# Blaizzy/mlx-audio

Measured on AMD Instinct MI355X. Metric: audio samples/sec + real-time factor, Kokoro-82M TTS, higher is better.
Workload: dtype bf16 weights x fp32 activations: vocoder convs = fp16 hi pass (v_mfma_f32_32x32x16_f16) + block-scaled FP4 (e2m1) lo pass (v_mfma_scale_f32_32x32x64_f8f6f4 cbsz / blgp 4, OCP MX: E8M0 scale per row x 32 channels / per output column), fp32 accumulate; front end bf16 hi+lo split; 1 GPU; Kokoro-82M bf16 TTS, tokens->waveform, canonical short sentence T=80 F=264 (6.6 s @ 24 kHz); utterances_per_gpu=64, global_batch=64, samples_per_utterance=158400, parallelism=utterance-dp1, precision_mode=6, wire=fp32

## Files before the change

include/mi355audio.h:

```cpp
#ifndef MI355AUDIO_H
#define MI355AUDIO_H

#include <stdint.h>

#ifdef __cplusplus
extern "C" {
#endif

#define MI355_OK 0
#define MI355_ERR_ARG (-1)
#define MI355_ERR_LAUNCH (-2)
#define MI355_ERR_UNSUPPORTED (-3)

const char* mi355_last_error(void);
int mi355_abi_version(void);
int mi355_device_info(int dev, char* name, int name_cap, int* cu_count, int* lds_bytes);

enum { MI355_ACT_NONE = 0, MI355_ACT_LEAKY = 1, MI355_ACT_SNAKE = 2, MI355_ACT_GELU = 3,
       MI355_ACT_ELU = 4,
       MI355_ACT_SILU = 5,
       MI355_ACT_GELU_TANH = 6,
       MI355_ACT_TANH = 7 };

typedef struct {
// ... 66 lines not shown
int mi355_pack_conv_weight_mx4_host(const float* w_host, int32_t Cout, int32_t K, int32_t Cin, uint8_t* out_host);

typedef struct {
  const float* x; int64_t x_bstride; int32_t ldx; int32_t C; int32_t L; const int32_t* lens;
  int32_t B;
  double* sums;
  const float* gb;
  int32_t gb_ld;
  float eps;
  float* scale; float* shift; int32_t out_ld;
  int32_t reuse_sums;
} mi355_adain_coef_args;
int mi355_adain_coef(const mi355_adain_coef_args* a, void* stream);

typedef struct {
  const float* partials; int64_t bstride;
  int32_t C; int32_t L; const int32_t* lens; int32_t B;
  const float* gb; int32_t gb_ld; float eps;
  float* scale; float* shift; int32_t out_ld;
} mi355_adain_partials_args;
int mi355_adain_from_partials(const mi355_adain_partials_args* a, void* stream);

typedef struct {
  const float* x; int64_t x_bstride; int32_t ldx;
  const float* res; int64_t res_bstride; int32_t ldr;
  int32_t C; int32_t L; const int32_t* lens; int32_t B;
  const float* weight; const float* bias;
  const float* ada_gb; int32_t ada_ld;
  float eps;
  int32_t post_act; float post_slope;
  float* y; int64_t y_bstride; int32_t ldy;
  int32_t y_split;
} mi355_layernorm_args;
int mi355_layernorm(const mi355_layernorm_args* a, void* stream);
int mi355_split16(const float* x, void* y, int64_t n, int32_t fmt, void* stream);

#define MI355_GN_PART_ELEMS 4096
typedef struct {
  const float* x; int64_t x_bstride; int32_t ldx;
  int32_t C; int32_t L; const int32_t* lens; int32_t B;
  double* partials; int64_t partials_bstride;
} mi355_group_norm_stats_args;
int mi355_group_norm_stats(const mi355_group_norm_stats_args* a, void* stream);

typedef struct {
  const void* partials; int64_t partials_bstride;
// ... 250 lines not shown
  const float* x; int64_t x_bstride; int32_t ldx; int32_t Fr; const int32_t* lens; int32_t B;
  int32_t n_fft; int32_t hop; const float* window;
  float* audio; int32_t ld_audio;
} mi355_istft_head_args;
int mi355_istft_head(const mi355_istft_head_args* a, void* stream);

typedef struct {
  const float* x; int64_t x_bstride; int32_t ldx; int32_t Cin; int32_t L; const int32_t* lens; int32_t B;
  const uint16_t* w; const float* bias; int32_t Cout; int32_t K; int32_t dil; int32_t pad;
  int32_t pre_act; float pre_slope; int32_t precision;
  int32_t n_fft; int32_t hop; const float* window;
  float* audio; int32_t ld_audio;
} mi355_conv_post_istft_args;
int mi355_conv_post_istft(const mi355_conv_post_istft_args* a, void* stream);

typedef struct {
  const float* x; int64_t x_bstride; int32_t ldx; int32_t Cin; int32_t L; const int32_t* lens; int32_t B;
  const uint16_t* w; const float* bias; int32_t Cout; int32_t K; int32_t u; int32_t p; int32_t row_off;
  float slope; int32_t precision;
  const float* res; int64_t res_bstride; int32_t ldr;
  float* y; int64_t y_bstride; int32_t ldy;
} mi355_upsample_polyphase_args;
int mi355_upsample_polyphase(const mi355_upsample_polyphase_args* a, void* stream);

typedef struct {
  const float* x; int32_t ldx; int32_t L; int32_t B;
  int32_t n_fft; int32_t hop; const float* window;
  int32_t pad_mode; int32_t n_frames;
  float* out;
} mi355_stft_args;
int mi355_stft(const mi355_stft_args* a, void* stream);

typedef struct {
  const float* x; int32_t ldx; int32_t L; int32_t B;
  int32_t n_fft; int32_t hop; const float* window; int32_t pad_mode; int32_t n_frames;
  const float* fb; int32_t n_mels; int32_t mode;
  float* out;
  float* gmax;
  float log_guard;
} mi355_logmel_args;
int mi355_logmel(const mi355_logmel_args* a, void* stream);
int mi355_logmel_finish(float* y, int64_t n_per_item, const float* gmax, int32_t B, void* stream);

typedef struct {
  const float* x; int32_t L;
  int32_t win; int32_t shift; int32_t pad; int32_t n_fft; int32_t n_frames;
// ... 426 lines not shown
```

mlx_audio_amd/csrc/norm.hip:

```cpp
#include "common.h"

namespace {

__global__ __launch_bounds__(256) void instnorm_partial_kernel(const mi355_adain_coef_args a, int rows_per_split) {
  __shared__ double red[2][32][33];
  const int tid = threadIdx.x, cg = tid & 7, rg = tid >> 3;
  const int b = blockIdx.z, c = blockIdx.x * 32 + cg * 4;
  const int len = a.lens ? a.lens[b] : a.L;
  const int r0 = blockIdx.y * rows_per_split;
  const int r1 = min(len, r0 + rows_per_split);
  double s[4] = {0, 0, 0, 0}, q[4] = {0, 0, 0, 0};
  const float* xb = a.x + (int64_t)b * a.x_bstride;
  if (c < a.C) {
    for (int l = r0 + rg; l < r1; l += 32) {
      const float4 v = *(const float4*)(xb + (int64_t)l * a.ldx + c);
      const float t[4] = {v.x, v.y, v.z, v.w};
#pragma unroll
      for (int i = 0; i < 4; ++i) { const double d = (double)t[i]; s[i] += d; q[i] += d * d; }
    }
  }
#pragma unroll
  for (int i = 0; i < 4; ++i) { red[0][rg][cg * 4 + i] = s[i]; red[1][rg][cg * 4 + i] = q[i]; }
  __syncthreads();
  if (tid < 64) {
// ... 89 lines not shown
        const float2 v0 = *(const float2*)(pb + (int64_t)e * estride), v1 = *(const float2*)(pb + (int64_t)(e + LPC) * estride);
        m2 += term(v0, e) + term(v1, e + LPC);
      }
      for (; e < nblk; e += LPC) m2 += term(*(const float2*)(pb + (int64_t)e * estride), e);
    }
  }
  red[cl][eg] = m2;
  __syncthreads();
  if (eg != 0 || c >= a.out_ld) return;
  float sc = 0.f, sh = 0.f;
  if (cok) {
    double q = 0.0;
    for (int j = 0; j < LPC; ++j) q += red[cl][j];
    double var = len > 0 ? q / (double)len : 0.0;
    if (var < 0) var = 0;
    const float rstd = 1.0f / sqrtf((float)var + a.eps);
    float g = 0.f, be = 0.f;
    if (a.gb) { g = a.gb[(int64_t)b * a.gb_ld + c]; be = a.gb[(int64_t)b * a.gb_ld + a.C + c]; }
    sc = (1.0f + g) * rstd;
    sh = be - (float)mean * sc;
  }
  a.scale[(int64_t)b * a.out_ld + c] = sc;
  a.shift[(int64_t)b * a.out_ld + c] = sh;
}

template <bool VEC, int NCH>
__global__ __launch_bounds__(256) void layernorm_kernel(const mi355_layernorm_args a) {
  const int lane = threadIdx.x & 63;
  const int64_t row = (int64_t)blockIdx.x * 4 + (threadIdx.x >> 6);
  if (row >= (int64_t)a.B * a.L) return;
  const int b = (int)(row / a.L), l = (int)(row - (int64_t)b * a.L);
  const int len = a.lens ? a.lens[b] : a.L;
  if (l >= len) return;
  const float* xr = a.x + (int64_t)b * a.x_bstride + (int64_t)l * a.ldx;
  const float* rr = a.res ? a.res + (int64_t)b * a.res_bstride + (int64_t)l * a.ldr : nullptr;
  float v[NCH][4];
  float s = 0.f;
  float4 w4[NCH], b4[NCH], g4[NCH], e4[NCH];
#pragma unroll
  for (int i = 0; i < NCH; ++i) {
    const int c = i * 256 + lane * 4;
    w4[i] = make_float4(1.f, 1.f, 1.f, 1.f); b4[i] = make_float4(0.f, 0.f, 0.f, 0.f); g4[i] = b4[i]; e4[i] = b4[i];
    if (c < a.C) {
      auto ld4 = [](const float* p) {
        if constexpr (VEC) return *(const float4*)p;
        else return make_float4(p[0], p[1], p[2], p[3]);
// ... 90 lines not shown
    MI355_CLEAR_ERROR();
    hipLaunchKernelGGL(instnorm_partial_kernel, dim3(cblocks, nsplit, a.B), dim3(256), 0, st, a, rows);
    MI355_LAUNCH_CHECK("instnorm_partial");
  }
  MI355_CLEAR_ERROR();
  hipLaunchKernelGGL(adain_finalize_kernel, dim3((a.out_ld + 127) / 128, a.B), dim3(128), 0, st, a);
  MI355_LAUNCH_CHECK("adain_finalize");
  return MI355_OK;
}

extern "C" int mi355_adain_from_partials(const mi355_adain_partials_args* ap, void* stream) {
  MI355_REQUIRE(ap && ap->partials && ap->scale && ap->shift, "adain_from_partials: null tensor");
  const mi355_adain_partials_args a = *ap;
  MI355_REQUIRE(a.B > 0 && a.C > 0 && a.L > 0 && a.out_ld >= a.C, "adain_from_partials: bad shape");
  MI355_CLEAR_ERROR();
  MI355_REQUIRE(a.bstride % 2 == 0 && ((uintptr_t)a.partials) % 8 == 0, "adain_from_partials: partials must be 8-byte aligned");
  static const int cpw_env = getenv("MI355_ADAIN_CPW") ? atoi(getenv("MI355_ADAIN_CPW")) : 0;
  if (a.B >= 8 && cpw_env != 4) hipLaunchKernelGGL(adain_from_partials_kernel<16>, dim3((a.out_ld + 15) / 16, a.B), dim3(256), 0, (hipStream_t)stream, a);
  else hipLaunchKernelGGL(adain_from_partials_kernel<4>, dim3((a.out_ld + 3) / 4, a.B), dim3(256), 0, (hipStream_t)stream, a);
  MI355_LAUNCH_CHECK("adain_from_partials");
  return MI355_OK;
}

extern "C" int mi355_layernorm(const mi355_layernorm_args* ap, void* stream) {
  MI355_REQUIRE(ap && ap->x && ap->y, "layernorm: null tensor");
  const mi355_layernorm_args a = *ap;
  MI355_REQUIRE(a.C > 0 && a.C <= 2048 && a.C % 4 == 0, "layernorm: C must be a multiple of 4 and <= 2048 (got %d)", a.C);
  MI355_REQUIRE(a.ldx % 4 == 0 && a.ldy % 4 == 0 && a.x_bstride % 4 == 0 && a.y_bstride % 4 == 0, "layernorm: strides must be multiples of 4");
  MI355_REQUIRE(!a.res || (a.ldr % 4 == 0 && a.res_bstride % 4 == 0), "layernorm: residual strides must be multiples of 4");
  MI355_REQUIRE(a.y_split == 0 || a.y_split == 2 || a.y_split == 4, "layernorm: y_split must be 0, 2 or 4");
  const int64_t rows = (int64_t)a.B * a.L;
  MI355_CLEAR_ERROR();
  const bool vec = ((uintptr_t)a.weight % 16 == 0) && ((uintptr_t)a.bias % 16 == 0) && ((uintptr_t)a.ada_gb % 16 == 0) && (a.ada_ld % 4 == 0);
  const dim3 grid((unsigned)((rows + 3) / 4));
  if (a.C <= 1024) {
    if (vec) hipLaunchKernelGGL((layernorm_kernel<true, 4>), grid, dim3(256), 0, (hipStream_t)stream, a);
    else hipLaunchKernelGGL((layernorm_kernel<false, 4>), grid, dim3(256), 0, (hipStream_t)stream, a);
  } else {
    if (vec) hipLaunchKernelGGL((layernorm_kernel<true, 8>), grid, dim3(256), 0, (hipStream_t)stream, a);
    else hipLaunchKernelGGL((layernorm_kernel<false, 8>), grid, dim3(256), 0, (hipStream_t)stream, a);
  }
  MI355_LAUNCH_CHECK("layernorm");
  return MI355_OK;
}
```

mlx_audio_amd/csrc/upsample_poly.hip:

```cpp
#include "conv_common.h"

using namespace mi355conv;

namespace {

constexpr int kUpThreads = 512;

template <int CIN, int COUT, int U, int MF, int NF>
__global__ __launch_bounds__(kUpThreads, 4) void upsample_poly_kernel(const mi355_upsample_polyphase_args a, const int nblk) {
  constexpr int H = MF * 32, R = H + 1, NCH = CIN / 32;
  constexpr int CHB = R * 64;
  constexpr int PLANE = NCH * CHB;
  constexpr int NFRAG = U * COUT / 32;
  constexpr int NG = NFRAG / NF;
  constexpr int NTp = ((U * COUT + 127) >> 7) << 2;
  constexpr int64_t WSTEP = (int64_t)NTp * 2048;
  constexpr int NS = NCH * 2;
  constexpr int DEPTH = 3;
  static_assert(NFRAG % NF == 0 && (COUT / 32) % NF == 0, "a column group lies inside one phase");
  static_assert(H * NCH * 8 % kUpThreads == 0, "whole passes over the first H window rows");
  extern __shared__ __attribute__((aligned(16))) char smem[];
  char* const A_hi = smem;
  char* const A_lo = smem + PLANE;

  const int tid = threadIdx.x;
  const int b = (int)blockIdx.x / nblk;
  const int m0 = ((int)blockIdx.x - b * nblk) * H;
  const int len_raw = a.lens ? a.lens[b] : a.L;
  const int len_in = len_raw < 0 ? 0 : (len_raw > a.L ? a.L : len_raw);
  if (m0 > len_in) return;
  const int len_up = len_in * U;

// ... 24 lines not shown
#pragma unroll
        for (int j = 0; j < 4; ++j) {
          float u = in[j] + 0.0f;
          const float m = u * slope;
          u = u > 0.f ? u : m;
          tt[j] = rowok ? u : 0.f;
        }
        uint2 ph, pl;
        ph.x = pack_bf16x2(tt[0], tt[1]);
        ph.y = pack_bf16x2(tt[2], tt[3]);
        const float h0 = __builtin_bit_cast(float, ph.x << 16), h1 = __builtin_bit_cast(float, ph.x & 0xffff0000u);
        const float h2 = __builtin_bit_cast(float, ph.y << 16), h3 = __builtin_bit_cast(float, ph.y & 0xffff0000u);
        pl.x = pack_bf16x2(tt[0] - h0, tt[1] - h1);
        pl.y = pack_bf16x2(tt[2] - h2, tt[3] - h3);
        const int addr = chunk * CHB + r * 64 + ((((c4 >> 3) ^ ((r >> 2) & 3))) << 4) + ((c4 & 4) << 1);
        *(uint2*)(A_hi + addr) = ph;
        *(uint2*)(A_lo + addr) = pl;
      }
    }
  }
  float* const yb = a.y + (int64_t)b * a.y_bstride;
  const float* const rb = a.res + (int64_t)b * a.res_bstride;
  if (a.row_off && m0 == 0) {
    for (int c = tid; c < COUT; c += kUpThreads) yb[c] = rb[c];
  }
  __syncthreads();

  const int wave = __builtin_amdgcn_readfirstlane(tid >> 6);
  for (int g = wave; g < NG; g += kUpThreads / 64) {
    int lane = tid & 63;
    asm volatile("" : "+v"(lane));
    const int hl = lane & 31, hh = lane >> 5;
    const int f0 = g * NF;
    const int phase = (f0 * 32) / COUT, oc0 = f0 * 32 - phase * COUT;
    const int nc0 = m0 * U + phase - a.p;
    const int len_up_c = len_up > 0 ? len_up : 1;

    f32x16 acc[MF][NF];
#pragma unroll
    for (int mf = 0; mf < MF; ++mf)
#pragma unroll
      for (int nf = 0; nf < NF; ++nf)
#pragma unroll
        for (int r = 0; r < 16; ++r) acc[mf][nf][r] = 0.f;

    const char* const wfrag = (const char*)a.w + (int64_t)f0 * 2048 + lane * 16;
    bf16x8 ring[DEPTH][2 * NF];
// ... 15 lines not shown
        bf16x8 ah[MF], al[MF];
#pragma unroll
        for (int mf = 0; mf < MF; ++mf) {
          const int row = mf * 32 + hl + tap;
          const int addr = chunk * CHB + row * 64 + (((kk * 2 + hh) ^ ((row >> 2) & 3)) << 4);
          ah[mf] = *(const bf16x8*)(A_hi + addr);
          al[mf] = *(const bf16x8*)(A_lo + addr);
        }
#pragma unroll
        for (int mf = 0; mf < MF; ++mf) {
#pragma unroll
          for (int nf = 0; nf < NF; ++nf) acc[mf][nf] = mfma16<2>(ah[mf], ring[sl % DEPTH][2 * nf + kk], acc[mf][nf]);
#pragma unroll
          for (int nf = 0; nf < NF; ++nf) acc[mf][nf] = mfma16<2>(al[mf], ring[sl % DEPTH][2 * nf + kk], acc[mf][nf]);
        }
      }
    }

    {
      const uint32_t col = (uint32_t)(oc0 + hl) * 4u, ypb = (uint32_t)a.ldy * 4u, rpb = (uint32_t)a.ldr * 4u;
      float bias[NF];
#pragma unroll
      for (int nf = 0; nf < NF; ++nf) bias[nf] = a.bias ? a.bias[oc0 + nf * 32 + hl] : 0.f;
#pragma unroll
      for (int mf = 0; mf < MF; ++mf) {
        float rv[NF][16];
#pragma unroll
        for (int r = 0; r < 16; ++r) {
          int nc = nc0 + (mf * 32 + (r & 3) + 8 * (r >> 2) + 4 * hh) * U;
          nc = nc < 0 ? 0 : (nc >= len_up_c ? len_up_c - 1 : nc);
          const uint32_t off = (uint32_t)(nc + a.row_off) * rpb + col;
#pragma unroll
          for (int nf = 0; nf < NF; ++nf) rv[nf][r] = *(const float*)((const char*)rb + (off + (uint32_t)(nf * 128)));
        }
#pragma unroll
        for (int r = 0; r < 16; ++r) {
          const int nc = nc0 + (mf * 32 + (r & 3) + 8 * (r >> 2) + 4 * hh) * U;
          if (nc >= 0 && nc < len_up) {
            const uint32_t off = (uint32_t)(nc + a.row_off) * ypb + col;
#pragma unroll
            for (int nf = 0; nf < NF; ++nf) *(float*)((char*)yb + (off + (uint32_t)(nf * 128))) = (acc[mf][nf][r] + bias[nf]) + rv[nf][r];
          }
        }
      }
    }
  }
}

template <int CIN, int COUT, int U, int MF, int NF>
int launch_up(const mi355_upsample_polyphase_args& a, hipStream_t st) {
  constexpr int H = MF * 32;
  constexpr int lds = 2 * (CIN / 32) * (H + 1) * 64;
  static bool attr_set = false;
  if (!attr_set) {
    hipError_t e = hipFuncSetAttribute((const void*)upsample_poly_kernel<CIN, COUT, U, MF, NF>, hipFuncAttributeMaxDynamicSharedMemorySize, lds);
    MI355_REQUIRE(e == hipSuccess, "upsample_polyphase: cannot reserve %d bytes of LDS: %s", lds, hipGetErrorString(e));
    attr_set = true;
  }
  const int nblk = (a.L + 1 + H - 1) / H;
  MI355_REQUIRE((int64_t)a.B * nblk < (int64_t)1 << 31, "upsample_polyphase: too many row blocks");
  MI355_CLEAR_ERROR();
  hipLaunchKernelGGL((upsample_poly_kernel<CIN, COUT, U, MF, NF>), dim3((unsigned)(a.B * nblk)), dim3(kUpThreads), lds, st, a, nblk);
  MI355_LAUNCH_CHECK("upsample_polyphase");
  return MI355_OK;
}

}

extern "C" int mi355_upsample_polyphase(const mi355_upsample_polyphase_args* ap, void* stream) {
  MI355_REQUIRE(ap && ap->x && ap->w && ap->res && ap->y, "upsample_polyphase: null tensor");
  const mi355_upsample_polyphase_args a = *ap;
  const bool s0 = a.Cin == 512 && a.Cout == 256 && a.u == 10, s1 = a.Cin == 256 && a.Cout == 128 && a.u == 6;
  if (!(s0 || s1) || a.K != 2 * a.u || a.p != (a.K - a.u) / 2 || a.precision != 2 || (a.row_off != 0 && a.row_off != 1)) {
    mi355_set_error("upsample_polyphase: unsupported shape (Cin=%d Cout=%d u=%d K=%d p=%d row_off=%d precision=%d)", a.Cin, a.Cout, a.u, a.K, a.p,
                    a.row_off, a.precision);
    return MI355_ERR_UNSUPPORTED;
  }
  const int64_t Lo = (int64_t)a.L * a.u + a.row_off;
  MI355_REQUIRE(a.B > 0 && a.L > 0 && a.ldx >= a.Cin && a.ldr >= a.Cout && a.ldy >= a.Cout, "upsample_polyphase: bad shape");
  MI355_REQUIRE(a.B == 1 || (a.x_bstride >= (int64_t)a.L * a.ldx && a.res_bstride >= Lo * a.ldr && a.y_bstride >= Lo * a.ldy), "upsample_polyphase: items overlap");
  MI355_REQUIRE(Lo * a.ldr < ((int64_t)1 << 29) && Lo * a.ldy < ((int64_t)1 << 29), "upsample_polyphase: an item's rows exceed the 32-bit byte offsets");
  MI355_REQUIRE((a.ldx & 3) == 0 && (a.x_bstride & 3) == 0 && (((uintptr_t)a.x | (uintptr_t)a.w) & 15) == 0, "upsample_polyphase: input rows must be 16-byte aligned");
  if (s0) return launch_up<512, 256, 10, 1, 2>(a, (hipStream_t)stream);
  return launch_up<256, 128, 6, 2, 1>(a, (hipStream_t)stream);
}
```

mlx_audio_amd/ops.py:

```python
from __future__ import annotations

import ctypes
import math
import os
from dataclasses import dataclass
from typing import Optional, Tuple

import numpy as np
import torch

from . import _lib

ACT_NONE, ACT_LEAKY, ACT_SNAKE, ACT_GELU, ACT_ELU, ACT_SILU, ACT_GELU_TANH, ACT_TANH = 0, 1, 2, 3, 4, 5, 6, 7

PROFILE = None


def _stream() -> int:
    return torch.cuda.current_stream().cuda_stream


def profile_finalize(entries):
    torch.cuda.synchronize()
    out = []
    for rows, cin, cout, k, dil, extra_reads, e0, e1 in entries:
        rows = int(rows)
        flops = 2.0 * rows * cout * k * cin
        byts = 4.0 * rows * (cin + cout * (1 + extra_reads)) + 2.0 * cout * k * cin
        out.append((flops, byts, e0, e1, (cin, cout, k, dil, rows)))
# ... 1550 lines not shown
            e0, e1 = torch.cuda.Event(enable_timing=True), torch.cuda.Event(enable_timing=True)
            e0.record()
            PROFILE.append(((L * B) if lens is None else lens.sum(), pc.cin, pc.cout, pc.k, dil, 0, e0, e1))
        _lib.call_struct("mi355_conv_post_istft", "mi355_conv_post_istft_args", _stream(), x=_ptr(x), x_bstride=xbs, ldx=ldx, Cin=pc.cin, L=L,
                         lens=_ptr(lens), B=B, w=_ptr(pc.w), bias=_ptr(pc.bias), Cout=pc.cout, K=pc.k, dil=dil, pad=pad, pre_act=pre_act,
                         pre_slope=pre_slope, precision=precision, n_fft=n_fft, hop=hop, window=_ptr(window), audio=_ptr(audio),
                         ld_audio=audio.stride(0))
        if PROFILE is not None:
            e1.record()
        return audio
    post = torch.empty((B, L, round_up(pc.cout, 4)), dtype=torch.float32, device=x.device)[:, :, :pc.cout]
    conv_gemm(x, pc, post, dil=dil, pad=pad, lens_in=lens, lens_out=lens, pre_act=pre_act, pre_slope=pre_slope, precision=precision, pre_fq=pre_fq)
    return istft_head(post, n_fft, hop, window, audio, lens=lens)


UPSAMPLE_POLY_SHAPES = {(512, 256, 10): 32, (256, 128, 6): 64}


def upsample_polyphase_eligible(pc: PackedConv, stride: int, *, pre_act: int = ACT_LEAKY, precision: int = 2, res=True, pre_fq=None) -> bool:
    return (pc.k == 2 and stride > 0 and pc.cout % stride == 0 and (pc.cin, pc.cout // stride, stride) in UPSAMPLE_POLY_SHAPES
            and pre_act == ACT_LEAKY and precision == 2 and not pc.f16 and not pc.mx and res is not None and pre_fq is None)


def upsample_polyphase(x: torch.Tensor, pc: PackedConv, res: torch.Tensor, y: torch.Tensor, stride: int, *, row_off: int = 0, lens=None,
                       pre_act: int = ACT_LEAKY, pre_slope: float = 0.1, precision: int = 2, pre_fq=None):
    B, L, _, xbs, ldx = _nlc(x)
    u = stride
    cout = pc.cout // u
    kfull = pc.k * u
    p = (kfull - u) // 2
    Lo = L * u + row_off
    assert y.shape[0] == B and y.shape[1] >= Lo and y.shape[2] == cout and res.shape[0] == B and res.shape[1] >= Lo and res.shape[2] == cout
    if upsample_polyphase_eligible(pc, u, pre_act=pre_act, precision=precision, res=res, pre_fq=pre_fq) and row_off in (0, 1):
        _, _, _, rbs, ldr = _nlc(res)
        _, _, _, ybs, ldy = _nlc(y)
        assert pc.w.numel() >= _lib.load().mi355_packed_conv_weight_elems(pc.cout, pc.k, pc.cin)
        if PROFILE is not None:
            e0, e1 = torch.cuda.Event(enable_timing=True), torch.cuda.Event(enable_timing=True)
            e0.record()
            PROFILE.append((((L + 1) * B) if lens is None else (lens + 1).sum(), pc.cin, pc.cout, pc.k, 1, 1, e0, e1))
        _lib.call_struct("mi355_upsample_polyphase", "mi355_upsample_polyphase_args", _stream(), x=_ptr(x), x_bstride=xbs, ldx=ldx, Cin=pc.cin, L=L,
                         lens=_ptr(lens), B=B, w=_ptr(pc.w), bias=_ptr(pc.bias), Cout=cout, K=kfull, u=u, p=p, row_off=row_off, slope=pre_slope,
                         precision=precision, res=_ptr(res), res_bstride=rbs, ldr=ldr, y=_ptr(y), y_bstride=ybs, ldy=ldy)
        if PROFILE is not None:
            e1.record()
        return y
    kp = pc.k
    conv_gemm(x, pc, y, pad=kp - 1, lout=L + kp - 1, lens_in=lens, lens_out=None if lens is None else lens + (kp - 1), pre_act=pre_act,
              pre_slope=pre_slope, res=res, precision=precision, pre_fq=pre_fq,
              up=dict(s=u, p=p, cout=cout, row_off=row_off, lout=L * u, lens=None if lens is None else lens * u))
    if row_off:
        y[:, :row_off, :].copy_(res[:, :row_off, :])
    return y


def stft_frames(x: torch.Tensor, n_fft: int, hop: int, window: torch.Tensor, pad_mode: int, n_frames: int):
    assert x.dim() == 2 and x.stride(1) == 1 and x.dtype == torch.float32
    B, L = x.shape
    out = torch.empty((B, n_frames, n_fft // 2 + 1, 2), dtype=torch.float32, device=x.device)
    _lib.call_struct("mi355_stft", "mi355_stft_args", _stream(), x=_ptr(x), ldx=x.stride(0), L=L, B=B, n_fft=n_fft, hop=hop,
                     window=_ptr(window), pad_mode=pad_mode, n_frames=n_frames, out=_ptr(out))
    return torch.view_as_complex(out)


def logmel(x: torch.Tensor, n_fft: int, hop: int, window: torch.Tensor, pad_mode: int, n_frames: int, fb: torch.Tensor,
           mode: int, log_guard: float = 0.0, fixed_max: Optional[float] = None):
    assert x.dim() == 2 and x.stride(1) == 1 and fb.is_contiguous()
    B, L = x.shape
    n_mels = fb.shape[0]
# ... 46 lines not shown
```

mlx_audio_amd/tts/models/kokoro/engine.py:

```python
from __future__ import annotations

import math
import os
from dataclasses import dataclass, field
from typing import Dict, List, Optional, Sequence

import numpy as np
import torch

from .... import ops
from ....ops import ACT_GELU, ACT_GELU_TANH, ACT_LEAKY, ACT_NONE, ACT_SNAKE, PackedConv, round_up


def fold_weight_norm(v: torch.Tensor, g: torch.Tensor, param_dtype: torch.dtype) -> torch.Tensor:
    v_ = v.to(param_dtype)
    g_ = g.to(param_dtype)
    axes = tuple(range(1, v_.dim()))
    nrm = torch.sqrt((v_ * v_).sum(dim=axes, keepdim=True))
    w = (v_ / (nrm + torch.tensor(1e-7, dtype=param_dtype))) * g_
    return w.to(torch.float32)


@dataclass
class _AdaIN:
# ... 122 lines not shown

    def _decoder_dims(self, config: dict):
        return 1024, 512, 64

    @staticmethod
    def default_precision(param_dtype, quant_modules: Sequence[str] = ()) -> int:
        if param_dtype == torch.float32:
            return 4
        return 6 if (param_dtype == torch.bfloat16 and not tuple(quant_modules)) else 2

    def __init__(self, weights: Dict[str, torch.Tensor], config: dict, device="cuda", param_dtype=torch.bfloat16,
                 precision: Optional[int] = None, quant_modules: Sequence[str] = ()):
        ops.require_gpu()
        self.cfg = config
        self.qmods = tuple(quant_modules)
        if precision is None:
            precision = self.default_precision(param_dtype, self.qmods)
        self.all_f16 = precision == 4
        self.cdim, self.gdim, self.adim = self._decoder_dims(config)
        self.dev = torch.device(device)
        self.pdt = param_dtype
        self.precision = precision
        self.fuse_stats = True
        self.fold_quant = os.environ.get("MI355_FOLD_QUANT", "1") != "0"
        self.ext_partials = os.environ.get("MI355_EXT_PARTIALS", "1") != "0"
        self.w = weights
        ist = config["istftnet"]
        self.rates = [int(r) for r in ist["upsample_rates"]]
        self.kers = [int(k) for k in ist["upsample_kernel_sizes"]]
        self.n_fft, self.hop = int(ist["gen_istft_n_fft"]), int(ist["gen_istft_hop_size"])
        self.total_up = int(np.prod(self.rates)) * self.hop
        self.rk = list(ist["resblock_kernel_sizes"])
        self.rd = [list(d) for d in ist["resblock_dilation_sizes"]]
        self.hid = config["hidden_dim"]
        self.sty = config["style_dim"]
        self.n_layer = config["n_layer"]
        self.pb = config["plbert"]
        self.bank_dec = _StyleBank()
        self.bank_pred = _StyleBank()
        self._load()

    def _t(self, name) -> torch.Tensor:
        return self.w[name].to(torch.float32)

    def _q(self, t: torch.Tensor) -> torch.Tensor:
        return t.to(self.pdt).to(torch.float32)
# ... 201 lines not shown
            pooled = self._new(B, Lo, round_up(blk.din, 32), zero=bool(self.qmods))[:, :, : blk.din]
            if self.qmods and self._isq(f"{nm}.pool"):
                xq = ops.fake_quant_u8(x, lens=lens, pre=(sc1, sh1), pre_act=ACT_LEAKY, pre_slope=0.2)
                one, zero = torch.ones_like(sc1), torch.zeros_like(sh1)
                ops.adain_pool_up2(xq, one, zero, 1.0, blk.pool_w, blk.pool_b, pooled, lens)
            else:
                ops.adain_pool_up2(x, sc1, sh1, 0.2, blk.pool_w, blk.pool_b, pooled, lens)
            self._convq(f"{nm}.conv1", pooled, blk.conv1, c1, pad=1, lens_in=lo, lens_out=lo, stats=st)
        else:
            self._convq(f"{nm}.conv1", x, blk.conv1, c1, pad=1, lens_in=lo, lens_out=lo, pre=(sc1, sh1), pre_act=ACT_LEAKY, pre_slope=0.2, stats=st)
        if st is not None:
            sc2, sh2 = ops.adain_from_partials(st, Lo, self._gb(gb_all, blk.norm2), lo)
        else:
            sc2, sh2 = ops.adain_coef(c1, self._gb(gb_all, blk.norm2), lo)
        if blk.conv1x1 is not None:
            short = self._new(B, L, blk.dout)
            self._convq(f"{nm}.conv1x1", x, blk.conv1x1, short, lens_in=lens, lens_out=lens, flatten=True)
        else:
            short = x
        self._convq(f"{nm}.conv2", c1, blk.conv2, out, pad=1, lens_in=lo, lens_out=lo, pre=(sc2, sh2), pre_act=ACT_LEAKY, pre_slope=0.2,
                    res=short, res_shift=1 if up else 0, out_scale=1.0 / math.sqrt(2.0))
        return out

    def _resblock1_fwd(self, rb: _ResBlock1, x, gb_all, lens, out=None, accumulate=False, out_scale=1.0, x_stats=None, x_sums=None):
        B, L, C = x.shape
        cur = x
        work = None
        tmp = self._new(B, L, C)
        fuse = self.fuse_stats
        st_cur = x_stats
        st_tmp = ops.new_stats(B, L, C, self.dev) if fuse else None
        st_work = ops.new_stats(B, L, C, self.dev) if fuse else None
        use_ext = bool(self.qmods) and self.fold_quant and self.ext_partials
        ex_cur = None
        ex_tmp = ops.new_ext(B, L, C, self.dev) if use_ext else None
        ex_work = ops.new_ext(B, L, C, self.dev) if use_ext else None
        for i, dl in enumerate(rb.dils):
            if fuse and st_cur is not None:
                sc, sh = ops.adain_from_partials(st_cur, L, self._gb(gb_all, rb.adain1[i]), lens)
            elif i == 0 and x_sums is not None:
                sc, sh = ops.adain_coef(cur, self._gb(gb_all, rb.adain1[i]), lens, sums=x_sums[0], reuse=x_sums[1])
            else:
                sc, sh = ops.adain_coef(cur, self._gb(gb_all, rb.adain1[i]), lens)
            _, ex_t = self._convq(f"{rb.name}.convs1.{i}", cur, rb.convs1[i], tmp, dil=dl, pad=(rb.k * dl - dl) // 2, lens_in=lens, lens_out=lens, pre=(sc, sh),
                                  pre_act=ACT_SNAKE, pre_alpha=rb.alpha1[i], stats=st_tmp, ext_in=ex_cur, ext_out=ex_tmp, ret_ext=True)
            if fuse:
                sc, sh = ops.adain_from_partials(st_tmp, L, self._gb(gb_all, rb.adain2[i]), lens)
            else:
                sc, sh = ops.adain_coef(tmp, self._gb(gb_all, rb.adain2[i]), lens)
            last = i == len(rb.dils) - 1
            if last and out is not None:
                dst, acc, scale = out, accumulate, out_scale
            else:
                if work is None:
                    work = self._new(B, L, C)
                dst, acc, scale = work, False, 1.0
            _, ex_w = self._convq(f"{rb.name}.convs2.{i}", tmp, rb.convs2[i], dst, pad=(rb.k - 1) // 2, lens_in=lens, lens_out=lens, pre=(sc, sh),
                                  pre_act=ACT_SNAKE, pre_alpha=rb.alpha2[i], res=cur, accumulate=acc, out_scale=scale,
                                  stats=st_work if (fuse and not last) else None, ext_in=ex_t, ext_out=None if last else ex_work, ret_ext=True)
            cur = dst
            st_cur = st_work if (fuse and not last) else None
# ... 215 lines not shown
                                  quant=bool(self.qmods) and self._isq(f"{g_n}.m_source.l_linear"), coarse_f32=self.coarse_f32)
        nb2 = self.n_fft + 2
        nbp = ops.round_up(nb2, 4)
        n_har = L2 * up // self.hop + 1
        har = self._new(B, n_har, nbp, zero=True)[:, :, :nb2]
        lens_samples = frames * (2 * up) if ragged else None
        ops.stft_magphase(har_src, self.n_fft, self.hop, self.window, har, lens=lens_samples)
        if "har" in overrides:
            har.copy_(overrides["har"].to(device=dev, dtype=torch.float32))
        lens_har = lens_samples // self.hop + 1 if ragged else None
        x = xg
        L = L2
        lens_x = lens_2f
        nk = len(self.rk)
        for i, (u, k) in enumerate(zip(self.rates, self.kers)):
            last = i + 1 == len(self.rates)
            cout = self.ups[i].cout // u
            Lo = L * u + (1 if last else 0)
            lens_o = (lens_x * u + (1 if last else 0)) if ragged else None
            xsrc = self._new(B, Lo, cout)
            har_i = har
            if self.qmods and self._isq(f"{g_n}.noise_convs.{i}"):
                har_i = ops.fake_quant_u8(har, y=self._new(B, n_har, nbp, zero=True)[:, :, :nb2], lens=lens_har)
            if not last:
                sf = int(np.prod(self.rates[i + 1:]))
                self._conv(har_i, self.noise_convs[i], xsrc, lens_in=lens_har, lens_out=lens_o,
                           flat=dict(ldx=sf * nbp, x_off=-((sf + 1) // 2) * nbp, channels=nbp))
            else:
                self._conv(har_i, self.noise_convs[i], xsrc, lens_in=lens_har, lens_out=lens_o)
            if return_intermediates:
                trace[f"nconv{i}"] = xsrc.clone()
            xsrc = self._resblock1_fwd(self.noise_res[i], xsrc, gb_dec, lens_o)
            if return_intermediates:
                trace[f"nres{i}"] = xsrc.clone()
            kp = k // u
            xu = self._new(B, Lo, cout)
            lens_gemm = (lens_x + (kp - 1)) if ragged else None
            lens_ct = (lens_x * u) if ragged else None
            if not (self.qmods and self._isq(f"{g_n}.ups.{i}")) and ops.upsample_polyphase_eligible(self.ups[i], u, precision=self._prec(self.ups[i])):
                ops.upsample_polyphase(x, self.ups[i], xsrc, xu, u, row_off=1 if last else 0, lens=lens_x, pre_slope=0.1, precision=self._prec(self.ups[i]))
            else:
                self._convq(f"{g_n}.ups.{i}", x, self.ups[i], xu, pad=kp - 1, lout=L + kp - 1, lens_in=lens_x, lens_out=lens_gemm, pre_act=ACT_LEAKY,
                            pre_slope=0.1, res=xsrc, up=dict(s=u, p=(k - u) // 2, cout=cout, row_off=1 if last else 0, lout=L * u, lens=lens_ct))
                if last:
                    xu[:, 0, :].copy_(xsrc[:, 0, :])
            if return_intermediates:
                trace[f"xu{i}"] = xu.clone()
            acc = self._new(B, Lo, cout)
            xu_sums = torch.empty(B * cout * 2, dtype=torch.float64, device=dev)
            for j in range(nk):
                self._resblock1_fwd(self.resblocks[i * nk + j], xu, gb_dec, lens_o, out=acc, accumulate=j > 0,
                                    out_scale=(1.0 / nk) if j == nk - 1 else 1.0, x_sums=(xu_sums, j > 0))
            x, L, lens_x = acc, Lo, lens_o
            if return_intermediates:
                trace[f"stage{i}"] = acc.clone()
        audio = self._new(B, (L - 1) * self.hop, zero=True)
        post = None
        if not return_intermediates and not (self.qmods and self._isq(f"{g_n}.conv_post")):
            ops.conv_post_istft(x, self.conv_post, self.n_fft, self.hop, self.window, audio, lens=lens_x, pre_slope=0.01, precision=self._prec(self.conv_post))
        else:
            post = self._new(B, L, round_up(nb2, 4))
            self._convq(f"{g_n}.conv_post", x, self.conv_post, post[:, :, :nb2], pad=3, lens_in=lens_x, lens_out=lens_x, pre_act=ACT_LEAKY, pre_slope=0.01)
            ops.istft_head(post[:, :, :nb2], self.n_fft, self.hop, self.window, audio, lens=lens_x)
        outs = [audio[b, : Fs[b] * 2 * up] for b in range(B)]
        durs = [dur[b, : Ts[b]] for b in range(B)]
        if return_intermediates:
            return outs, durs, dict(d=d, en=en, f0=f0_curve, n=n_curve, asr=asr, t_en=t_en, dur_raw=dur_raw, har_src=har_src,
                                    har=har, bert=h, xg=xg, post=post[:, :, :nb2], dec3=xg, **trace)
        return outs, durs
```

Before: 202.2 million samples/s.

## Fuse AdaIN statistics into polyphase upsample epilogue and last noise conv

The polyphase upsample kernel gains a STATS variant whose epilogue computes per-phase, per-block channel sums and M2 partials of its output and writes them to a partials buffer. A new kernel merges those partials with a Chan-style combine into AdaIN scale/shift for up to four resblocks in one launch. This replaces the separate full reread of the upsampled tensor by adain_coef. The last noise conv also emits stats so the noise resblock can skip its own reduction pass. In exchange the upsample epilogue carries extra registers and shuffles, which may lower occupancy, and the statistics are now accumulated in fp32 partials instead of fp64 sums.

```diff
diff --git a/include/mi355audio.h b/include/mi355audio.h
--- a/include/mi355audio.h
+++ b/include/mi355audio.h
@@ -112,6 +112,17 @@
 int mi355_adain_from_partials(const mi355_adain_partials_args* a, void* stream);
 
 typedef struct {
+  const float* partials; int64_t bstride;
+  int32_t C; int32_t L; const int32_t* lens; int32_t B;
+  int32_t u; int32_t p; int32_t H; int32_t row_off;
+  int32_t nset; float eps; int32_t gb_ld; int32_t out_ld;
+  const float* gb0; const float* gb1; const float* gb2; const float* gb3;
+  float* scale0; float* scale1; float* scale2; float* scale3;
+  float* shift0; float* shift1; float* shift2; float* shift3;
+} mi355_adain_phase_partials_args;
+int mi355_adain_from_phase_partials(const mi355_adain_phase_partials_args* a, void* stream);
+
+typedef struct {
   const float* x; int64_t x_bstride; int32_t ldx;
   const float* res; int64_t res_bstride; int32_t ldr;
   int32_t C; int32_t L; const int32_t* lens; int32_t B;
@@ -408,6 +419,16 @@
   float* y; int64_t y_bstride; int32_t ldy;
 } mi355_upsample_polyphase_args;
 int mi355_upsample_polyphase(const mi355_upsample_polyphase_args* a, void* stream);
+
+typedef struct {
+  const float* x; int64_t x_bstride; int32_t ldx; int32_t Cin; int32_t L; const int32_t* lens; int32_t B;
+  const uint16_t* w; const float* bias; int32_t Cout; int32_t K; int32_t u; int32_t p; int32_t row_off;
+  float slope; int32_t precision;
+  const float* res; int64_t res_bstride; int32_t ldr;
+  float* y; int64_t y_bstride; int32_t ldy;
+  float* stats_partial; int64_t stats_bstride;
+} mi355_upsample_polyphase_stats_args;
+int mi355_upsample_polyphase_stats(const mi355_upsample_polyphase_stats_args* a, void* stream);
 
 typedef struct {
   const float* x; int32_t ldx; int32_t L; int32_t B;
diff --git a/mlx_audio_amd/csrc/norm.hip b/mlx_audio_amd/csrc/norm.hip
--- a/mlx_audio_amd/csrc/norm.hip
+++ b/mlx_audio_amd/csrc/norm.hip
@@ -135,6 +135,102 @@
   }
   a.scale[(int64_t)b * a.out_ld + c] = sc;
   a.shift[(int64_t)b * a.out_ld + c] = sh;
+}
+
+constexpr int kPhaseCPW = 16, kPhaseLPC = 256 / kPhaseCPW;
+__global__ __launch_bounds__(256) void adain_from_phase_partials_kernel(const mi355_adain_phase_partials_args a) {
+  __shared__ double red[kPhaseCPW][kPhaseLPC + 1];
+  const int cl = threadIdx.x % kPhaseCPW, eg = threadIdx.x / kPhaseCPW;
+  const int c = blockIdx.x * kPhaseCPW + cl, b = blockIdx.y;
+  const int len_raw = a.lens ? a.lens[b] : a.L;
+  const int len_in = len_raw < 0 ? 0 : (len_raw > a.L ? a.L : len_raw);
+  const int len_up = len_in * a.u;
+  const int n = len_up + a.row_off;
+  const int nphase = (len_in / a.H + 1) * a.u;
+  const int nent = nphase + a.row_off;
+  const int pad_e = (a.L / a.H + 1) * a.u;
+  const bool cok = c < a.C;
+  const float* pb = a.partials + (int64_t)b * a.bstride + (int64_t)(cok ? c : 0) * 2;
+  const int64_t estride = (int64_t)a.C * 2;
+  auto count = [&](const int e) {
+    if (e >= nphase) return 1;
+    const int blk = e / a.u, phase = e - blk * a.u;
+    const int lo = max(blk * a.H, phase >= a.p ? 0 : 1);
+    const int hi = min(blk * a.H + a.H, (len_up + a.p - phase + a.u - 1) / a.u);
+    return hi > lo ? hi - lo : 0;
+  };
+  auto entry = [&](const int e) { return *(const float2*)(pb + (int64_t)(e >= nphase ? pad_e : e) * estride); };
+  const bool keep = nent <= kAdainKeep * kPhaseLPC;
+  float2 kept[kAdainKeep];
+  int cnt[kAdainKeep];
+  double s = 0.0;
+  if (cok) {
+    if (keep) {
+#pragma unroll
+      for (int j = 0; j < kAdainKeep; ++j) {
+        const int e = eg + j * kPhaseLPC;
+        kept[j] = entry(e < nent ? e : nent - 1);
+      }
+#pragma unroll
+      for (int j = 0; j < kAdainKeep; ++j) {
+        const int e = eg + j * kPhaseLPC;
+        cnt[j] = e < nent ? count(e) : 0;
+        kept[j].x = cnt[j] > 0 ? kept[j].x : 0.f;
+        kept[j].y = cnt[j] > 0 ? kept[j].y : 0.f;
+      }
+#pragma unroll
+      for (int j = 0; j < kAdainKeep; ++j) s += (double)kept[j].x;
+    } else {
+      for (int e = eg; e < nent; e += kPhaseLPC) {
+        const float2 v = entry(e);
+        s += count(e) > 0 ? (double)v.x : 0.0;
+      }
+    }
+  }
+  red[cl][eg] = s;
+  __syncthreads();
+  double tot = 0.0;
+  for (int j = 0; j < kPhaseLPC; ++j) tot += red[cl][j];
+  const double mean = n > 0 ? tot / (double)n : 0.0;
+  __syncthreads();
+  double m2 = 0.0;
+  if (cok) {
+    auto term = [&](const float2 sv, const int k) {
+      const double d = (double)sv.x / (double)k - mean;
+      return (double)sv.y + d * d * (double)k;
+    };
+    if (keep) {
+#pragma unroll
+      for (int j = 0; j < kAdainKeep; ++j)
+        if (cnt[j] > 0) m2 += term(kept[j], cnt[j]);
+    } else {
+      for (int e = eg; e < nent; e += kPhaseLPC) {
+        const float2 v = entry(e);
+        const int k = count(e);
+        if (k > 0) m2 += term(v, k);
+      }
+    }
+  }
+  red[cl][eg] = m2;
+  __syncthreads();
+  if (eg >= a.nset || c >= a.out_ld) return;
+  const float* const gb = eg == 0 ? a.gb0 : (eg == 1 ? a.gb1 : (eg == 2 ? a.gb2 : a.gb3));
+  float* const scale = eg == 0 ? a.scale0 : (eg == 1 ? a.scale1 : (eg == 2 ? a.scale2 : a.scale3));
+  float* const shift = eg == 0 ? a.shift0 : (eg == 1 ? a.shift1 : (eg == 2 ? a.shift2 : a.shift3));
+  float sc = 0.f, sh = 0.f;
+  if (cok) {
+    double q = 0.0;
+    for (int j = 0; j < kPhaseLPC; ++j) q += red[cl][j];
+    double var = n > 0 ? q / (double)n : 0.0;
+    if (var < 0) var = 0;
+    const float rstd = 1.0f / sqrtf((float)var + a.eps);
+    float g = 0.f, be = 0.f;
+    if (gb) { g = gb[(int64_t)b * a.gb_ld + c]; be = gb[(int64_t)b * a.gb_ld + a.C + c]; }
+    sc = (1.0f + g) * rstd;
+    sh = be - (float)mean * sc;
+  }
+  scale[(int64_t)b * a.out_ld + c] = sc;
+  shift[(int64_t)b * a.out_ld + c] = sh;
 }
 
 template <bool VEC, int NCH>
@@ -271,6 +367,25 @@
   return MI355_OK;
 }
 
+extern "C" int mi355_adain_from_phase_partials(const mi355_adain_phase_partials_args* ap, void* stream) {
+  MI355_REQUIRE(ap && ap->partials, "adain_from_phase_partials: null tensor");
+  const mi355_adain_phase_partials_args a = *ap;
+  MI355_REQUIRE(a.nset >= 1 && a.nset <= 4, "adain_from_phase_partials: nset must be 1 .. 4 (got %d)", a.nset);
+  const float* const sc[4] = {a.scale0, a.scale1, a.scale2, a.scale3};
+  const float* const sh[4] = {a.shift0, a.shift1, a.shift2, a.shift3};
+  for (int i = 0; i < a.nset; ++i) MI355_REQUIRE(sc[i] && sh[i], "adain_from_phase_partials: null scale / shift of set %d", i);
+  MI355_REQUIRE(a.B > 0 && a.C > 0 && a.L > 0 && a.out_ld >= a.C, "adain_from_phase_partials: bad shape");
+  MI355_REQUIRE(a.u > 0 && a.H > 0 && a.p >= 0 && a.p < a.u && (a.row_off == 0 || a.row_off == 1), "adain_from_phase_partials: bad geometry (u=%d p=%d H=%d row_off=%d)",
+                a.u, a.p, a.H, a.row_off);
+  MI355_REQUIRE((int64_t)a.L * a.u < ((int64_t)1 << 30), "adain_from_phase_partials: too many rows");
+  MI355_REQUIRE(a.bstride % 2 == 0 && ((uintptr_t)a.partials) % 8 == 0, "adain_from_phase_partials: partials must be 8-byte aligned");
+  MI355_REQUIRE(a.B == 1 || a.bstride >= ((int64_t)(a.L / a.H + 1) * a.u + a.row_off) * a.C * 2, "adain_from_phase_partials: the items' partials overlap");
+  MI355_CLEAR_ERROR();
+  hipLaunchKernelGGL(adain_from_phase_partials_kernel, dim3((a.out_ld + kPhaseCPW - 1) / kPhaseCPW, a.B), dim3(256), 0, (hipStream_t)stream, a);
+  MI355_LAUNCH_CHECK("adain_from_phase_partials");
+  return MI355_OK;
+}
+
 extern "C" int mi355_layernorm(const mi355_layernorm_args* ap, void* stream) {
   MI355_REQUIRE(ap && ap->x && ap->y, "layernorm: null tensor");
   const mi355_layernorm_args a = *ap;
diff --git a/mlx_audio_amd/csrc/upsample_poly.hip b/mlx_audio_amd/csrc/upsample_poly.hip
--- a/mlx_audio_amd/csrc/upsample_poly.hip
+++ b/mlx_audio_amd/csrc/upsample_poly.hip
@@ -1,4 +1,5 @@
 #include "conv_common.h"
+#include <type_traits>
 
 using namespace mi355conv;
 
@@ -6,8 +7,11 @@
 
 constexpr int kUpThreads = 512;
 
-template <int CIN, int COUT, int U, int MF, int NF>
-__global__ __launch_bounds__(kUpThreads, 4) void upsample_poly_kernel(const mi355_upsample_polyphase_args a, const int nblk) {
+template <bool STATS>
+using up_args_t = std::conditional_t<STATS, mi355_upsample_polyphase_stats_args, mi355_upsample_polyphase_args>;
+
+template <int CIN, int COUT, int U, int MF, int NF, bool STATS>
+__global__ __launch_bounds__(kUpThreads, 4) void upsample_poly_kernel(const up_args_t<STATS> a, const int nblk) {
   constexpr int H = MF * 32, R = H + 1, NCH = CIN / 32;
   constexpr int CHB = R * 64;
   constexpr int PLANE = NCH * CHB;
@@ -78,7 +82,10 @@
   float* const yb = a.y + (int64_t)b * a.y_bstride;
   const float* const rb = a.res + (int64_t)b * a.res_bstride;
   if (a.row_off && m0 == 0) {
-    for (int c = tid; c < COUT; c += kUpThreads) yb[c] = rb[c];
+    for (int c = tid; c < COUT; c += kUpThreads) {
+      yb[c] = rb[c];
+      if constexpr (STATS) *(float2*)(a.stats_partial + (int64_t)b * a.stats_bstride + ((int64_t)nblk * U * COUT + c) * 2) = make_float2(rb[c], 0.f);
+    }
   }
   __syncthreads();
 
@@ -140,6 +147,8 @@
       float bias[NF];
 #pragma unroll
       for (int nf = 0; nf < NF; ++nf) bias[nf] = a.bias ? a.bias[oc0 + nf * 32 + hl] : 0.f;
+      [[maybe_unused]] uint32_t okm = 0;
+      [[maybe_unused]] float sv[STATS ? MF : 1][NF][16];
 #pragma unroll
       for (int mf = 0; mf < MF; ++mf) {
         float rv[NF][16];
@@ -151,43 +160,81 @@
 #pragma unroll
           for (int nf = 0; nf < NF; ++nf) rv[nf][r] = *(const float*)((const char*)rb + (off + (uint32_t)(nf * 128)));
         }
+        if constexpr (STATS) {
+#pragma unroll
+          for (int r = 0; r < 16; ++r) {
+            const int nc = nc0 + (mf * 32 + (r & 3) + 8 * (r >> 2) + 4 * hh) * U;
+            okm |= (nc >= 0 && nc < len_up) ? 1u << (mf * 16 + r) : 0u;
+#pragma unroll
+            for (int nf = 0; nf < NF; ++nf) sv[mf][nf][r] = (acc[mf][nf][r] + bias[nf]) + rv[nf][r];
+          }
+        }
 #pragma unroll
         for (int r = 0; r < 16; ++r) {
           const int nc = nc0 + (mf * 32 + (r & 3) + 8 * (r >> 2) + 4 * hh) * U;
           if (nc >= 0 && nc < len_up) {
             const uint32_t off = (uint32_t)(nc + a.row_off) * ypb + col;
 #pragma unroll
-            for (int nf = 0; nf < NF; ++nf) *(float*)((char*)yb + (off + (uint32_t)(nf * 128))) = (acc[mf][nf][r] + bias[nf]) + rv[nf][r];
+            for (int nf = 0; nf < NF; ++nf) {
+              float v = (acc[mf][nf][r] + bias[nf]) + rv[nf][r];
+              if constexpr (STATS) v = sv[mf][nf][r];
+              *(float*)((char*)yb + (off + (uint32_t)(nf * 128))) = v;
+            }
           }
         }
       }
-    }
-  }
-}
-
-template <int CIN, int COUT, int U, int MF, int NF>
-int launch_up(const mi355_upsample_polyphase_args& a, hipStream_t st) {
+      if constexpr (STATS) {
+        const float cl = (float)__popc(okm);
+        const float icl = okm ? 1.0f / cl : 0.f;
+        float* const sp = a.stats_partial + (int64_t)b * a.stats_bstride + ((int64_t)((m0 / H) * U + phase) * COUT + oc0 + hl) * 2;
+#pragma unroll
+        for (int nf = 0; nf < NF; ++nf) {
+          float sl = 0.f;
+#pragma unroll
+          for (int mf = 0; mf < MF; ++mf)
+#pragma unroll
+            for (int r = 0; r < 16; ++r) sl += ((okm >> (mf * 16 + r)) & 1u) ? sv[mf][nf][r] : 0.f;
+          const float ml = sl * icl;
+          float vl = 0.f;
+#pragma unroll
+          for (int mf = 0; mf < MF; ++mf)
+#pragma unroll
+            for (int r = 0; r < 16; ++r) {
+              const float d = sv[mf][nf][r] - ml;
+              vl += ((okm >> (mf * 16 + r)) & 1u) ? d * d : 0.f;
+            }
+          const float cp = __shfl_xor(cl, 32, 64), sq = __shfl_xor(sl, 32, 64), mp = __shfl_xor(ml, 32, 64), vp = __shfl_xor(vl, 32, 64);
+          const float ct = cl + cp, dm = mp - ml;
+          const float m2 = vl + vp + (ct > 0.f ? dm * dm * cl * cp / ct : 0.f);
+          if (hh == 0) *(float2*)(sp + nf * 64) = make_float2(sl + sq, m2);
+        }
+      }
+    }
+  }
+}
+
+template <int CIN, int COUT, int U, int MF, int NF, bool STATS>
+int launch_up(const up_args_t<STATS>& a, hipStream_t st) {
   constexpr int H = MF * 32;
   constexpr int lds = 2 * (CIN / 32) * (H + 1) * 64;
   static bool attr_set = false;
   if (!attr_set) {
-    hipError_t e = hipFuncSetAttribute((const void*)upsample_poly_kernel<CIN, COUT, U, MF, NF>, hipFuncAttributeMaxDynamicSharedMemorySize, lds);
+    hipError_t e = hipFuncSetAttribute((const void*)upsample_poly_kernel<CIN, COUT, U, MF, NF, STATS>, hipFuncAttributeMaxDynamicSharedMemorySize, lds);
     MI355_REQUIRE(e == hipSuccess, "upsample_polyphase: cannot reserve %d bytes of LDS: %s", lds, hipGetErrorString(e));
     attr_set = true;
   }
   const int nblk = (a.L + 1 + H - 1) / H;
   MI355_REQUIRE((int64_t)a.B * nblk < (int64_t)1 << 31, "upsample_polyphase: too many row blocks");
   MI355_CLEAR_ERROR();
-  hipLaunchKernelGGL((upsample_poly_kernel<CIN, COUT, U, MF, NF>), dim3((unsigned)(a.B * nblk)), dim3(kUpThreads), lds, st, a, nblk);
+  hipLaunchKernelGGL((upsample_poly_kernel<CIN, COUT, U, MF, NF, STATS>),dim3((unsigned)(a.B * nblk)), dim3(kUpThreads), lds, st, a, nblk);
   MI355_LAUNCH_CHECK("upsample_polyphase");
   return MI355_OK;
 }
 
-}
-
-extern "C" int mi355_upsample_polyphase(const mi355_upsample_polyphase_args* ap, void* stream) {
+template <bool STATS>
+int upsample_entry(const up_args_t<STATS>* ap, void* stream) {
   MI355_REQUIRE(ap && ap->x && ap->w && ap->res && ap->y, "upsample_polyphase: null tensor");
-  const mi355_upsample_polyphase_args a = *ap;
+  const up_args_t<STATS> a = *ap;
   const bool s0 = a.Cin == 512 && a.Cout == 256 && a.u == 10, s1 = a.Cin == 256 && a.Cout == 128 && a.u == 6;
   if (!(s0 || s1) || a.K != 2 * a.u || a.p != (a.K - a.u) / 2 || a.precision != 2 || (a.row_off != 0 && a.row_off != 1)) {
     mi355_set_error("upsample_polyphase: unsupported shape (Cin=%d Cout=%d u=%d K=%d p=%d row_off=%d precision=%d)", a.Cin, a.Cout, a.u, a.K, a.p,
@@ -199,6 +246,17 @@
   MI355_REQUIRE(a.B == 1 || (a.x_bstride >= (int64_t)a.L * a.ldx && a.res_bstride >= Lo * a.ldr && a.y_bstride >= Lo * a.ldy), "upsample_polyphase: items overlap");
   MI355_REQUIRE(Lo * a.ldr < ((int64_t)1 << 29) && Lo * a.ldy < ((int64_t)1 << 29), "upsample_polyphase: an item's rows exceed the 32-bit byte offsets");
   MI355_REQUIRE((a.ldx & 3) == 0 && (a.x_bstride & 3) == 0 && (((uintptr_t)a.x | (uintptr_t)a.w) & 15) == 0, "upsample_polyphase: input rows must be 16-byte aligned");
-  if (s0) return launch_up<512, 256, 10, 1, 2>(a, (hipStream_t)stream);
-  return launch_up<256, 128, 6, 2, 1>(a, (hipStream_t)stream);
-}
+  if constexpr (STATS) {
+    const int64_t need = ((int64_t)(a.L / (s0 ? 32 : 64) + 1) * a.u + a.row_off) * a.Cout * 2;
+    MI355_REQUIRE(a.stats_partial && ((uintptr_t)a.stats_partial) % 8 == 0 && a.stats_bstride % 2 == 0, "upsample_polyphase_stats: stats_partial must be set and 8-byte aligned");
+    MI355_REQUIRE(a.B == 1 || a.stats_bstride >= need, "upsample_polyphase_stats: the items' partials overlap");
+  }
+  if (s0) return launch_up<512, 256, 10, 1, 2, STATS>(a, (hipStream_t)stream);
+  return launch_up<256, 128, 6, 2, 1, STATS>(a, (hipStream_t)stream);
+}
+
+}
+
+extern "C" int mi355_upsample_polyphase(const mi355_upsample_polyphase_args* ap, void* stream) { return upsample_entry<false>(ap, stream); }
+
+extern "C" int mi355_upsample_polyphase_stats(const mi355_upsample_polyphase_stats_args* ap, void* stream) { return upsample_entry<true>(ap, stream); }
diff --git a/mlx_audio_amd/ops.py b/mlx_audio_amd/ops.py
--- a/mlx_audio_amd/ops.py
+++ b/mlx_audio_amd/ops.py
@@ -4,7 +4,7 @@
 import math
 import os
 from dataclasses import dataclass
-from typing import Optional, Tuple
+from typing import Optional, Sequence, Tuple
 
 import numpy as np
 import torch
@@ -1601,8 +1601,33 @@
             and pre_act == ACT_LEAKY and precision == 2 and not pc.f16 and not pc.mx and res is not None and pre_fq is None)
 
 
+def new_phase_stats(B: int, L: int, pc: PackedConv, stride: int, row_off: int, device) -> torch.Tensor:
+    cout = pc.cout // stride
+    H = UPSAMPLE_POLY_SHAPES[(pc.cin, cout, stride)]
+    return torch.empty((B, (L // H + 1) * stride + row_off, cout, 2), dtype=torch.float32, device=device)
+
+
+def adain_from_phase_partials(stats: torch.Tensor, L: int, pc: PackedConv, stride: int, row_off: int, gbs: Sequence[Optional[torch.Tensor]],
+                              lens: Optional[torch.Tensor] = None, eps: float = 1e-5):
+    B, nent, C, _ = stats.shape
+    u = stride
+    H = UPSAMPLE_POLY_SHAPES[(pc.cin, C, u)]
+    assert stats.is_contiguous() and nent == (L // H + 1) * u + row_off and 1 <= len(gbs) <= 4
+    lds = {gb.stride(0) for gb in gbs if gb is not None}
+    assert len(lds) <= 1
+    cp = round_up(C, 32)
+    out = [(torch.empty((B, cp), dtype=torch.float32, device=stats.device), torch.empty((B, cp), dtype=torch.float32, device=stats.device)) for _ in gbs]
+    kw = {}
+    for i, (gb, (sc, sh)) in enumerate(zip(gbs, out)):
+        kw[f"gb{i}"], kw[f"scale{i}"], kw[f"shift{i}"] = _ptr(gb), _ptr(sc), _ptr(sh)
+    _lib.call_struct("mi355_adain_from_phase_partials", "mi355_adain_phase_partials_args", _stream(), partials=_ptr(stats), bstride=stats.stride(0),
+                     C=C, L=L, lens=_ptr(lens), B=B, u=u, p=(pc.k * u - u) // 2, H=H, row_off=row_off, nset=len(gbs), eps=eps,
+                     gb_ld=lds.pop() if lds else 0, out_ld=cp, **kw)
+    return out
+
+
 def upsample_polyphase(x: torch.Tensor, pc: PackedConv, res: torch.Tensor, y: torch.Tensor, stride: int, *, row_off: int = 0, lens=None,
-                       pre_act: int = ACT_LEAKY, pre_slope: float = 0.1, precision: int = 2, pre_fq=None):
+                       pre_act: int = ACT_LEAKY, pre_slope: float = 0.1, precision: int = 2, pre_fq=None, stats: Optional[torch.Tensor] = None):
     B, L, _, xbs, ldx = _nlc(x)
     u = stride
     cout = pc.cout // u
@@ -1618,12 +1643,19 @@
             e0, e1 = torch.cuda.Event(enable_timing=True), torch.cuda.Event(enable_timing=True)
             e0.record()
             PROFILE.append((((L + 1) * B) if lens is None else (lens + 1).sum(), pc.cin, pc.cout, pc.k, 1, 1, e0, e1))
-        _lib.call_struct("mi355_upsample_polyphase", "mi355_upsample_polyphase_args", _stream(), x=_ptr(x), x_bstride=xbs, ldx=ldx, Cin=pc.cin, L=L,
-                         lens=_ptr(lens), B=B, w=_ptr(pc.w), bias=_ptr(pc.bias), Cout=cout, K=kfull, u=u, p=p, row_off=row_off, slope=pre_slope,
-                         precision=precision, res=_ptr(res), res_bstride=rbs, ldr=ldr, y=_ptr(y), y_bstride=ybs, ldy=ldy)
+        kw = dict(x=_ptr(x), x_bstride=xbs, ldx=ldx, Cin=pc.cin, L=L, lens=_ptr(lens), B=B, w=_ptr(pc.w), bias=_ptr(pc.bias), Cout=cout, K=kfull, u=u,
+                  p=p, row_off=row_off, slope=pre_slope, precision=precision, res=_ptr(res), res_bstride=rbs, ldr=ldr, y=_ptr(y), y_bstride=ybs, ldy=ldy)
+        if stats is not None:
+            assert stats.is_contiguous() and tuple(stats.shape) == ((B, (L // UPSAMPLE_POLY_SHAPES[(pc.cin, cout, u)] + 1) * u + row_off, cout, 2))
+            _lib.call_struct("mi355_upsample_polyphase_stats", "mi355_upsample_polyphase_stats_args", _stream(), stats_partial=_ptr(stats),
+                             stats_bstride=stats.stride(0), **kw)
+        else:
+            _lib.call_struct("mi355_upsample_polyphase", "mi355_upsample_polyphase_args", _stream(), **kw)
         if PROFILE is not None:
             e1.record()
         return y
+    if stats is not None:
+        raise _lib.Mi355Error("upsample_polyphase(stats=...): only the dedicated kernel writes phase partials, and it does not take this up-sampler")
     kp = pc.k
     conv_gemm(x, pc, y, pad=kp - 1, lout=L + kp - 1, lens_in=lens, lens_out=None if lens is None else lens + (kp - 1), pre_act=pre_act,
               pre_slope=pre_slope, res=res, precision=precision, pre_fq=pre_fq,
diff --git a/mlx_audio_amd/tts/models/kokoro/engine.py b/mlx_audio_amd/tts/models/kokoro/engine.py
--- a/mlx_audio_amd/tts/models/kokoro/engine.py
+++ b/mlx_audio_amd/tts/models/kokoro/engine.py
@@ -168,6 +168,7 @@
         self.pdt = param_dtype
         self.precision = precision
         self.fuse_stats = True
+        self.stage_stats = True
         self.fold_quant = os.environ.get("MI355_FOLD_QUANT", "1") != "0"
         self.ext_partials = os.environ.get("MI355_EXT_PARTIALS", "1") != "0"
         self.w = weights
@@ -415,7 +416,7 @@
                     res=short, res_shift=1 if up else 0, out_scale=1.0 / math.sqrt(2.0))
         return out
 
-    def _resblock1_fwd(self, rb: _ResBlock1, x, gb_all, lens, out=None, accumulate=False, out_scale=1.0, x_stats=None, x_sums=None):
+    def _resblock1_fwd(self, rb: _ResBlock1, x, gb_all, lens, out=None, accumulate=False, out_scale=1.0, x_stats=None, x_sums=None, x_coef=None):
         B, L, C = x.shape
         cur = x
         work = None
@@ -429,7 +430,9 @@
         ex_tmp = ops.new_ext(B, L, C, self.dev) if use_ext else None
         ex_work = ops.new_ext(B, L, C, self.dev) if use_ext else None
         for i, dl in enumerate(rb.dils):
-            if fuse and st_cur is not None:
+            if i == 0 and x_coef is not None:
+                sc, sh = x_coef
+            elif fuse and st_cur is not None:
                 sc, sh = ops.adain_from_partials(st_cur, L, self._gb(gb_all, rb.adain1[i]), lens)
             elif i == 0 and x_sums is not None:
                 sc, sh = ops.adain_coef(cur, self._gb(gb_all, rb.adain1[i]), lens, sums=x_sums[0], reuse=x_sums[1])
@@ -691,23 +694,32 @@
             har_i = har
             if self.qmods and self._isq(f"{g_n}.noise_convs.{i}"):
                 har_i = ops.fake_quant_u8(har, y=self._new(B, n_har, nbp, zero=True)[:, :, :nb2], lens=lens_har)
+            st_src = None
             if not last:
                 sf = int(np.prod(self.rates[i + 1:]))
                 self._conv(har_i, self.noise_convs[i], xsrc, lens_in=lens_har, lens_out=lens_o,
                            flat=dict(ldx=sf * nbp, x_off=-((sf + 1) // 2) * nbp, channels=nbp))
             else:
-                self._conv(har_i, self.noise_convs[i], xsrc, lens_in=lens_har, lens_out=lens_o)
+                if self.stage_stats and self.fuse_stats and not self.qmods:
+                    st_src = ops.new_stats(B, Lo, cout, dev)
+                self._conv(har_i, self.noise_convs[i], xsrc, lens_in=lens_har, lens_out=lens_o, stats=st_src)
             if return_intermediates:
                 trace[f"nconv{i}"] = xsrc.clone()
-            xsrc = self._resblock1_fwd(self.noise_res[i], xsrc, gb_dec, lens_o)
+            xsrc = self._resblock1_fwd(self.noise_res[i], xsrc, gb_dec, lens_o, x_stats=st_src)
             if return_intermediates:
                 trace[f"nres{i}"] = xsrc.clone()
             kp = k // u
             xu = self._new(B, Lo, cout)
             lens_gemm = (lens_x + (kp - 1)) if ragged else None
             lens_ct = (lens_x * u) if ragged else None
+            xu_coef = None
             if not (self.qmods and self._isq(f"{g_n}.ups.{i}")) and ops.upsample_polyphase_eligible(self.ups[i], u, precision=self._prec(self.ups[i])):
-                ops.upsample_polyphase(x, self.ups[i], xsrc, xu, u, row_off=1 if last else 0, lens=lens_x, pre_slope=0.1, precision=self._prec(self.ups[i]))
+                ro = 1 if last else 0
+                st_xu = ops.new_phase_stats(B, L, self.ups[i], u, ro, dev) if (self.stage_stats and nk <= 4) else None
+                ops.upsample_polyphase(x, self.ups[i], xsrc, xu, u, row_off=ro, lens=lens_x, pre_slope=0.1, precision=self._prec(self.ups[i]), stats=st_xu)
+                if st_xu is not None:
+                    xu_coef = ops.adain_from_phase_partials(st_xu, L, self.ups[i], u, ro, [self._gb(gb_dec, self.resblocks[i * nk + j].adain1[0]) for j in range(nk)],
+                                                            lens=lens_x)
             else:
                 self._convq(f"{g_n}.ups.{i}", x, self.ups[i], xu, pad=kp - 1, lout=L + kp - 1, lens_in=lens_x, lens_out=lens_gemm, pre_act=ACT_LEAKY,
                             pre_slope=0.1, res=xsrc, up=dict(s=u, p=(k - u) // 2, cout=cout, row_off=1 if last else 0, lout=L * u, lens=lens_ct))
@@ -716,10 +728,11 @@
             if return_intermediates:
                 trace[f"xu{i}"] = xu.clone()
             acc = self._new(B, Lo, cout)
-            xu_sums = torch.empty(B * cout * 2, dtype=torch.float64, device=dev)
+            xu_sums = torch.empty(B * cout * 2, dtype=torch.float64, device=dev) if xu_coef is None else None
             for j in range(nk):
                 self._resblock1_fwd(self.resblocks[i * nk + j], xu, gb_dec, lens_o, out=acc, accumulate=j > 0,
-                                    out_scale=(1.0 / nk) if j == nk - 1 else 1.0, x_sums=(xu_sums, j > 0))
+                                    out_scale=(1.0 / nk) if j == nk - 1 else 1.0, x_sums=None if xu_coef is not None else (xu_sums, j > 0),
+                                    x_coef=None if xu_coef is None else xu_coef[j])
             x, L, lens_x = acc, Lo, lens_o
             if return_intermediates:
                 trace[f"stage{i}"] = acc.clone()
```

Result: slower. 199.3 million samples/s (-1.4%).
